# GATB/leon

Hardware: AMD Instinct MI355X
Metric: compressed input MB/s (DNA encode path) (higher is better)
Workload: dtype u64

## Files before the change

### leon_amd/csrc/capi.hip

```cpp
#include "../../include/leon_dna.h"
#include "kernels.h"
#include "host_rc.h"
#include "staging.h"
#include "host_blocks.h"

#include "prim.h"

#include <algorithm>
#include <atomic>
#include <chrono>
#include <cstdio>
#include <cstdlib>
#include <cstring>
#include <functional>
#include <mutex>
#include <string>
#include <thread>
#include <vector>

using namespace leon;

namespace {

thread_local std::string g_create_error;
// ... 820 lines not shown
            if (int rc = resolve_window(w0, w1)) return rc;
            while (w1 < n && packed_upto < std::min(n, w1 + W)) { if (int rc = pack_next_group()) return rc; }
            c->stats.resolve_windows++;
        }
        if (pending.buf >= 0) { HIPCHK(c, spin_sync(s)); hand_over(); }
        if (knobs.trace_resolve) {
            unsigned long long t[12];
            HIPCHK(c, hipMemcpy(t, d_trace, sizeof t, hipMemcpyDeviceToHost));
            const char* cls[3] = {"found an anchor of the dictionary", "went on to propose its own", "no anchor at all"};
            for (int j = 0; j < 3; j++)
                if (t[4 * j]) fprintf(stderr, "[leon resolve] k_lookup_cand, reads that %-34s: %10llu reads, per read %.1f filter probes, %.1f dictionary probes behind a filter maybe, %.1f k-mers through the bloom\n",
                                      cls[j], t[4 * j], (double)t[4 * j + 1] / t[4 * j], (double)t[4 * j + 2] / t[4 * j], (double)t[4 * j + 3] / t[4 * j]);
        }
        HIPCHK(c, hipGetLastError());
        HIPCHK(c, hipEventRecord(c->ev[2], s));
        mark("resolution launched to its end");
        return LEON_OK;
    }
    int resolve_window(uint64_t w0, uint64_t w1) {
        if (int rc = dict_reserve(c, c->n_keys + (w1 - w0))) return rc;
        HIPCHK(c, hipMemsetAsync(counters, 0, 8, s));
        HIPCHK(c, hipMemsetAsync(c->wbits.p, 0, (1ull << WBITS_LOG2) / 8, s));
        HIPCHK(c, hipMemsetAsync(c->pbits.p, 0, (1ull << WBITS_LOG2) / 8, s));
        if (!share_lookups) launch_lookup_cand(s, R, c->B, c->d_rv16, c->D, V, w0, w1, first_read_index, lists[0], counters, d_trace);
        else if (int rc = look_up_shared(w0, w1)) return rc;
        HIPCHK(c, hipMemcpyAsync(d_hist, counters, 4, hipMemcpyDeviceToDevice, s));
        uint32_t cnt0 = 0;
        if (int rc = fixpoint_rounds(w0, w1, cnt0)) return rc;
        hint = std::max<uint32_t>(2 * cnt0, 4096);
        if (cnt0 > 0) { if (int rc = settle(w0, w1)) return rc; }
        launch_finalize_reads(s, R, c->D, V, w0, w1);
        return LEON_OK;
    }
    int look_up_shared(uint64_t w0, uint64_t w1) {
        const uint32_t Wn = c->shard_world; const uint64_t P = (w1 - w0 + Wn - 1) / Wn;
        auto run_of = [&](uint32_t r, uint64_t& a, uint64_t& b) { a = std::min(w1, w0 + (uint64_t)r * P); b = std::min(w1, a + P); };
        HIPCHK(c, c->xch_res.ensure((uint64_t)Wn * P * 8)); uint64_t* xres = c->xch_res.as<uint64_t>();
        uint64_t s0 = 0, s1 = 0; run_of(c->shard_rank, s0, s1);
        launch_lookup_cand(s, R, c->B, c->d_rv16, c->D, V, s0, s1, first_read_index, lists[0], counters, d_trace, xres, w0, false);
        HIPCHK(c, hipStreamSynchronize(s));
        const auto t_l0 = std::chrono::steady_clock::now();
        if (c->xch_mode == LEON_XCH_BY_ANCHOR) {
            if (c->gather_fn(c->gather_user, xres, P * 8, Wn)) return fail(c, LEON_E_STATE, "the gather callback returned non-zero");
            HIPCHK(c, hipSetDevice(c->device));
            lk_call_ms += ms_since(t_l0);
        } else {
            for (uint32_t r = 0; r < Wn; r++) {
                if (r == c->shard_rank) continue;
                uint64_t a = 0, b = 0; run_of(r, a, b);
                launch_lookup_cand(s, R, c->B, c->d_rv16, c->D, V, a, b, first_read_index, lists[0], counters, nullptr, xres, w0, true);
            }
            HIPCHK(c, hipStreamSynchronize(s));
            lk_emul_ms += ms_since(t_l0);
        }
        launch_lookup_apply(s, R, c->D, V, w0, w1, s0, s1, first_read_index, xres, lists[0], counters);
        return LEON_OK;
    }
    int fixpoint_rounds(uint64_t w0, uint64_t w1, uint32_t& cnt0) {
        int cur = 0;
        uint32_t n_hist = 1;
        bool first_wait = true;
        for (uint32_t ahead = knobs.rounds_ahead;; ahead = kRoundsMore) {
            for (uint32_t r = 0; r < ahead && n_hist < kHist; r++) {
                const int nxt = cur ^ 1;
                const uint32_t h = std::max<uint32_t>(hint >> (2 * (n_hist - 1) < 31 ? 2 * (n_hist - 1) : 31), 4096);
                HIPCHK(c, hipMemsetAsync(counters + nxt, 0, 4, s));
                launch_check(s, R, c->D, V, first_read_index, lists[cur], counters + cur, h, lists[nxt], counters + nxt);
                HIPCHK(c, hipMemcpyAsync(d_hist + n_hist, counters + nxt, 4, hipMemcpyDeviceToDevice, s));
                launch_reset_tent(s, c->D, V, lists[cur], counters + cur, h);
                launch_propose(s, c->D, V, first_read_index, lists[nxt], counters + nxt, h);
                cur = nxt; n_hist++;
            }
            HIPCHK(c, hipMemcpyAsync(c->h_rb + 8, d_hist, n_hist * 4, hipMemcpyDeviceToHost, s));
// ... 51 lines not shown
            launch_chain_prep(s, true, R, c->D, V, first_read_index, w0, clist + c0, nc, c0, rank, cnt, own, rows, ent, om, late, dep, xdep);
            if (launch_chain_seq(s, nc, cnt, own, dep, xdep, rows, ent, c->chain_ins.as<unsigned long long>(), d_ctrace))
                return fail(c, LEON_E_HIP, "the sequential resolution pass could not be launched (its LDS request was refused)");
            launch_chain_apply(s, c->D, V, first_read_index, clist + c0, nc, c->chain_ins.as<unsigned long long>(), k);
            HIPCHK(c, hipGetLastError());
        }
        { const uint32_t c_last = (left - 1) / CH * CH; launch_chain_repropose(s, c->D, V, first_read_index, clist + c_last, left - c_last, nullptr, 0); }
        HIPCHK(c, hipEventRecord(c->chain_ev[2 * n_chain_ev + 1], s));
        n_chain_ev++;
        c->stats.resolve_chain_reads += left; c->stats.resolve_chain_windows++;
        if (knobs.trace_chain) {
            unsigned long long t[8];
            HIPCHK(c, hipStreamSynchronize(s));
            HIPCHK(c, hipMemcpy(t, d_ctrace, sizeof t, hipMemcpyDeviceToHost));
            float cms = 0; (void)hipEventElapsedTime(&cms, c->chain_ev[2 * n_chain_ev - 2], c->chain_ev[2 * n_chain_ev - 1]);
            fprintf(stderr, "[leon chain] window [%llu, %llu): %u reads left by the rounds; %llu steps of 64, %.2f ballot iterations and %.1f entry rows per step, %llu inserters; %.2f ms; per step the settler waited %.0f (tester: %.0f), settled + published %.0f ticks of s_memtime\n",
                    (unsigned long long)w0, (unsigned long long)w1, left, t[0], t[0] ? (double)t[1] / t[0] : 0.0, t[0] ? (double)t[2] / t[0] : 0.0, t[3], cms,
                    t[0] ? (double)t[4] / t[0] : 0.0, t[0] ? (double)t[5] / t[0] : 0.0, t[0] ? (double)t[6] / t[0] : 0.0);
        }
        return LEON_OK;
    }
    int settle(uint64_t w0, uint64_t w1) {
        launch_final_pos(s, R, c->D, V, w0, w1, first_read_index);
        launch_ins_flags(s, V, w0, w1);
        HIPCHK(c, prim::ExclusiveSum(c->cub_tmp.p, scan_tmp, V.ins_flag, c->rank.as<uint32_t>(), w1 - w0, s));
        HIPCHK(c, hipMemcpyAsync(c->h_rb + 0, c->rank.as<uint32_t>() + (w1 - w0 - 1), 4, hipMemcpyDeviceToHost, s));
        HIPCHK(c, hipMemcpyAsync(c->h_rb + 1, V.ins_flag + (w1 - w0 - 1), 4, hipMemcpyDeviceToHost, s));
        HIPCHK(c, hipMemcpyAsync(c->h_rb + 2, c->d_nkeys, 8, hipMemcpyDeviceToHost, s));
        HIPCHK(c, spin_sync(s));
        const uint64_t n_new = (uint64_t)(uint32_t)c->h_rb[0] + (uint32_t)c->h_rb[1];
        c->n_keys = c->h_rb[2];
        if (c->n_anchors + n_new > 0xFFFFFFFFull) return fail(c, LEON_E_OVERFLOW, "more than 2^32 anchors");
        if ((c->n_anchors + n_new) * 8 * KW > c->anchor_kmers.cap) {
            TmpBuf nb;
            HIPCHK(c, nb.ensure(std::max<uint64_t>((c->n_anchors + n_new) * 2, 1024) * 8 * KW));
            if (c->n_anchors) HIPCHK(c, hipMemcpyAsync(nb.p, c->anchor_kmers.p, c->n_anchors * 8 * KW, hipMemcpyDeviceToDevice, s));
            HIPCHK(c, hipStreamSynchronize(s));
            std::swap(static_cast<DevBuf&>(nb).p, c->anchor_kmers.p);
            std::swap(static_cast<DevBuf&>(nb).cap, c->anchor_kmers.cap);
        }
        launch_assign_addr(s, c->D, V, w0, w1, c->rank.as<uint32_t>(), c->n_anchors, c->anchor_kmers.as<uint64_t>(), k);
        if (n_new && c->shard_rank == 0 && !(c->cfg.flags & LEON_F_DICT_ON_DEVICE)) {
            HIPCHK(c, hipMemcpyAsync(c->h_anchor[anchor_buf], c->anchor_kmers.as<uint64_t>() + c->n_anchors * KW, n_new * 8 * KW, hipMemcpyDeviceToHost, s));
            pending.buf = anchor_buf; pending.n = n_new;
            anchor_buf ^= 1;
            if (w0 == 0) {
                HIPCHK(c, spin_sync(s));
// ... 1263 lines not shown
```

### leon_amd/csrc/dna_kernels.hip

```cpp
#include "kernels.h"

namespace leon {

static inline uint32_t grid_for(uint64_t items, uint32_t per_block, uint32_t cap = 256 * 32) {
    uint64_t g = (items + per_block - 1) / per_block;
    if (g < 1) g = 1;
    if (g > cap) g = cap;
    return (uint32_t)g;
}
#define DISPATCH_K(k, CALL) do { if ((k) >= 32) { typedef u128 K; CALL; } else { typedef uint64_t K; CALL; } } while (0)

template <typename K>
__global__ void __launch_bounds__(256) k_bloom_insert(BloomDev B, const uint16_t* rv16g, const uint64_t* kmers, uint64_t n) {
    __shared__ uint16_t rv16[256];
    load_rv16(rv16, rv16g);
    uint32_t* words = (uint32_t*)B.bits;
    for (uint64_t i = blockIdx.x * (uint64_t)blockDim.x + threadIdx.x; i < n; i += (uint64_t)gridDim.x * blockDim.x) {
        BloomKeys Kk;
        const uint32_t pv = bloom_item_keys<K>(B, rv16, load_kmer<K>(kmers + i * KT<K>::W), Kk);
        for (uint32_t h = 0; h < B.n_hash; h++) {
            uint64_t pos = Kk.racine + Kk.key[h] + pv;
            atomicOr(&words[pos >> 5], 1u << (pos & 31));
        }
    }
// ... 256 lines not shown
template <typename K> __device__ inline K canon_at(const uint32_t* pk, uint32_t p, uint32_t k) {
    const K km = kmer_at<K>(pk, p, k);
    const K rc = revcomp(km, k);
    return rc < km ? rc : km;
}

template <typename K> __device__ inline K fwd_from_words16(uint32_t words, uint32_t gbase, uint32_t base, uint32_t p, uint32_t k);
template <> __device__ inline uint64_t fwd_from_words16<uint64_t>(uint32_t words, uint32_t gbase, uint32_t base, uint32_t p, uint32_t k) {
    const int d = (int)(gbase + (p >> 4) - (base >> 4));
    return kmer_from3((uint32_t)__shfl((int)words, d), (uint32_t)__shfl((int)words, d + 1), (uint32_t)__shfl((int)words, d + 2), p & 15, k);
}
template <> __device__ inline u128 fwd_from_words16<u128>(uint32_t words, uint32_t gbase, uint32_t base, uint32_t p, uint32_t k) {
    const int d = (int)(gbase + (p >> 4) - (base >> 4));
    return kmer_from5((uint32_t)__shfl((int)words, d), (uint32_t)__shfl((int)words, d + 1), (uint32_t)__shfl((int)words, d + 2),
                      (uint32_t)__shfl((int)words, d + 3), (uint32_t)__shfl((int)words, d + 4), p & 15, k);
}
template <typename K> __device__ inline K canon_from_words16(uint32_t words, uint32_t gbase, uint32_t base, uint32_t p, uint32_t k) {
    const K km = fwd_from_words16<K>(words, gbase, base, p, k);
    const K rc = revcomp(km, k);
    return rc < km ? rc : km;
}

template <typename K, bool TRACE>
__global__ void __launch_bounds__(256, (KT<K>::W == 2 ? 5 : 8)) k_lookup_cand(ReadsDev R, BloomDev B, const uint16_t* rv16g, DictDev D, ResolveDev V,
                                                    uint64_t w0, uint64_t w1, uint64_t first_global,
                                                    uint32_t* ulist, uint32_t* ucount, unsigned long long* trace,
                                                    uint64_t* xres, uint64_t xbase, uint32_t dry) {
    __shared__ uint16_t rv16[256];
    load_rv16(rv16, rv16g);
    const uint32_t lane = lane_id(), k = R.k;
    const uint32_t grp = lane >> 4, l = lane & 15, gbase = grp * 16;
    const uint64_t wave = (blockIdx.x * (uint64_t)blockDim.x + threadIdx.x) >> 6;
    const uint64_t nwaves = ((uint64_t)gridDim.x * blockDim.x) >> 6;
    enum : uint32_t { PH_LOOKUP = 0, PH_SEG_A = 1, PH_SEG_B = 2, PH_SEG_C = 3, PH_DONE = 4 };
    __shared__ uint32_t lists[4][64];
    uint32_t* my_list = lists[threadIdx.x >> 6];
    uint32_t n_list = 0, n_created = 0;
    auto flush_list = [&]() {
        if (n_list) {
            uint32_t at = 0;
            if (lane == 0) at = atomicAdd(ucount, n_list);
            at = (uint32_t)__shfl((int)at, 0);
            __builtin_amdgcn_wave_barrier();
            if (lane < n_list) ulist[at + lane] = my_list[lane];
            __builtin_amdgcn_wave_barrier();
        }
        if (n_created && lane == 0) atomicAdd(D.n_keys, (unsigned long long)n_created);
        n_list = 0; n_created = 0;
    };
    uint32_t t_filter = 0, t_dict = 0, t_bloom = 0;
    unsigned long long tr[12] = {0, 0, 0, 0, 0, 0, 0, 0, 0, 0, 0, 0};
    auto trace_done = [&](uint32_t cls) { if (TRACE && l == 0) { tr[cls * 4] += 1; tr[cls * 4 + 1] += t_filter; tr[cls * 4 + 2] += t_dict; tr[cls * 4 + 3] += t_bloom; } t_filter = t_dict = t_bloom = 0; };
    uint64_t i = w0 + 4 * wave + grp;
    bool have = false, started = false, exhausted = false;
    uint32_t len = 0, nk = 0, iMin = 0, iMax = 0, phase = PH_DONE, base = 0, limit = 0;
    uint64_t g = 0;
    const uint32_t* pk = R.packed;
    const uint32_t mm_m = D.mm_m, mm_P = D.mm_P, mm_c = D.mm_c;
    const uint64_t* const fwords = (const uint64_t*)D.fbits;
    MinLevels prev = {~0u, ~0u, ~0u, ~0u, ~0u};
    for (;;) {
        if (phase == PH_DONE && !exhausted) {
            if (started) i += 4 * nwaves;
            started = true;
            have = i < w1;
            exhausted = !have;
            if (have) {
                len = R.len[i];
                g = first_global + i;
                pk = R.packed + 2 * R.slot_off[i];
                nk = len >= k ? len - k + 1 : 0;
                iMin = nk / 2; iMax = nk / 2 + 10 > nk ? nk : nk / 2 + 10;
                base = 0; limit = nk;
                if (nk) phase = PH_LOOKUP;
                else { if (l == 0) { if (!dry) V.status[i] = ST_NOANCHOR; if (xres) xres[i - xbase] = ST_NOANCHOR; } trace_done(2); }
            }
        }
        if (!__any(have)) break;
        {
            const bool active = phase != PH_DONE;
            if (active && base >= limit) {
                if (phase == PH_LOOKUP) { phase = PH_SEG_A; base = iMin; limit = iMax; }
                else if (phase == PH_SEG_A) { phase = PH_SEG_B; base = 0; limit = iMin; }
                else if (phase == PH_SEG_B) { phase = PH_SEG_C; base = iMax; limit = nk; }
                else { phase = PH_DONE; if (l == 0) { if (!dry) V.status[i] = ST_NOANCHOR; if (xres) xres[i - xbase] = ST_NOANCHOR; } trace_done(2); }
            }
            const bool run = phase != PH_DONE && base < limit;
            const uint32_t p = base + l;
            const bool valid = run && p < limit;
            const uint32_t words = (run && l < 8) ? pk[(base >> 4) + l] : 0u;
            const K km = fwd_from_words16<K>(words, gbase, base, valid ? p : (run ? limit - 1 : 0), k);
            const K rck = revcomp(km, k);
            const K cn = rck < km ? rck : km;
            const bool look = run && phase == PH_LOOKUP;
            if (look && base == 0) {
                prev = MinLevels{~0u, ~0u, ~0u, ~0u, ~0u};
                for (int r = mm_P == 32 ? 1 : 0; r >= 0; r--) {
                    const int x = (int)(mm_c + mm_P - 1) - 16 * (r + 1) + (int)l;
                    const uint32_t xc = x > 0 ? (uint32_t)x : 0u;
                    const uint32_t w0 = (uint32_t)__shfl((int)words, (int)(gbase + (xc >> 4))), w1 = (uint32_t)__shfl((int)words, (int)(gbase + (xc >> 4) + 1));
                    const uint32_t mm = (uint32_t)((((((uint64_t)w0) << 32) | w1) << (2 * (xc & 15))) >> (64 - 2 * mm_m));
                    prev = sliding_levels(x >= (int)mm_c && xc + mm_m <= len ? mmer_hash(mm, mm_m) : ~0u, prev);
                }
            }
            const MinLevels cur = sliding_levels(look && valid ? mmer_hash(mmer_of(km, k, mm_m, mm_c + mm_P - 1), mm_m) : ~0u, prev);
            const uint32_t hmin = window_minimum(cur, prev, mm_P);
            if (look) prev = cur;
            bool hit = false; uint32_t slot = 0xFFFFFFFFu;
            if (valid) {
                if (phase == PH_LOOKUP) {
                    const uint64_t fb = filter_bits(cn);
                    const bool maybe = (fwords[filter_word(D, hmin)] & fb) == fb;
                    if (maybe) { uint64_t fin = IDX_INF; slot = dict_find(D, cn, fin); hit = slot != 0xFFFFFFFFu && fin < g; }
                    if (TRACE) {
                        const uint32_t nf = (uint32_t)__popcll(__ballot(true) >> gbase & 0xFFFFull), nd = (uint32_t)__popcll(__ballot(maybe) >> gbase & 0xFFFFull);
                        t_filter += nf; t_dict += nd;
                    }
                }
                else { hit = bloom_contains<K>(B, rv16, cn); if (TRACE) t_bloom += (uint32_t)__popcll(__ballot(true) >> gbase & 0xFFFFull); }
            }
            const unsigned long long bal = __ballot(hit);
            const uint32_t gb = (uint32_t)(bal >> gbase) & 0xFFFFu;
            bool want_insert = false; uint32_t cpos = 0;
            if (run) {
                if (gb) {
                    const uint32_t f = (uint32_t)__builtin_ctz(gb);
                    const uint32_t hs = __shfl(slot, (int)(gbase + f));
                    if (phase == PH_LOOKUP) {
                        if (l == 0) {
                            if (!dry) { V.status[i] = ST_HIT; V.hit_pos[i] = base + f; V.hit_slot[i] = hs; }
                            if (xres) xres[i - xbase] = ((uint64_t)(base + f) << 8) | ST_HIT;
                        }
                        trace_done(0);
                    } else {
                        want_insert = (l == 0) && !dry; cpos = base + f;
                        if (l == 0 && xres) xres[i - xbase] = ((uint64_t)cpos << 8) | ST_UNRESOLVED;
                        trace_done(1);
                    }
                    phase = PH_DONE;
                } else base += 16;
            }
            bool created = false;
            uint32_t sl = 0;
            for (uint32_t q = 0; q < 4; q++) {
                if (want_insert && grp == q) {
                    const K ck = canon_at<K>(pk, cpos, k);
                    sl = dict_find_or_insert<true>(D, ck, created);
                    atomicMin((unsigned long long*)tent_ptr(D, sl), (unsigned long long)g);
                    const uint32_t pb = window_bit(ck);
                    atomicOr(&D.pbits[pb >> 5], 1u << (pb & 31));
                    V.status[i] = ST_UNRESOLVED; V.cand_pos[i] = cpos; V.cand_slot[i] = sl;
                }
            }
            const unsigned long long wm = __ballot(want_insert);
            if (wm) {
                if (want_insert) my_list[n_list + (uint32_t)__popcll(wm & ((1ull << lane) - 1))] = (uint32_t)i;
                n_list += (uint32_t)__popcll(wm);
                n_created += (uint32_t)__popcll(__ballot(created));
                if (n_list > 64 - 4) flush_list();
            }
        }
    }
    flush_list();
    if (TRACE) {
        for (uint32_t j = 0; j < 12; j++) {
            unsigned long long v = tr[j];
            for (int d = 1; d < 64; d <<= 1) v += __shfl_xor(v, d);
            if (lane == 0 && v) atomicAdd(trace + j, v);
        }
    }
}
void launch_lookup_cand(hipStream_t s, ReadsDev R, BloomDev B, const uint16_t* rv16, DictDev D, ResolveDev V,
                        uint64_t w0, uint64_t w1, uint64_t first_global, uint32_t* ulist, uint32_t* ucount, unsigned long long* trace,
                        uint64_t* xres, uint64_t xbase, bool dry) {
    if (w1 <= w0) return;
    if (trace && !dry) { DISPATCH_K(R.k, hipLaunchKernelGGL((k_lookup_cand<K, true>), dim3(grid_for(w1 - w0, 16, 256 * 16)), dim3(256), 0, s, R, B, rv16, D, V, w0, w1,
                                                           first_global, ulist, ucount, trace, xres, xbase, 0u)); return; }
    const uint32_t per_cu = [] { const char* e = getenv("LEON_LOOKUP_BLOCKS_PER_CU"); const int v = e ? atoi(e) : 0; return v > 0 && v <= 1024 ? (uint32_t)v : 16u; }();
    DISPATCH_K(R.k, hipLaunchKernelGGL((k_lookup_cand<K, false>), dim3(grid_for(w1 - w0, 16, 256 * per_cu)), dim3(256), 0, s, R, B, rv16, D, V, w0, w1,
                                       first_global, ulist, ucount, trace, xres, xbase, dry ? 1u : 0u));
}

template <typename K>
__global__ void __launch_bounds__(256) k_lookup_apply(ReadsDev R, DictDev D, ResolveDev V, uint64_t w0, uint64_t w1, uint64_t s0, uint64_t s1,
                                                     uint64_t first_global, const uint64_t* xres, uint32_t* ulist, uint32_t* ucount) {
    __shared__ uint32_t wave_n[4], wave_new[4], block_at;
    const uint32_t lane = lane_id(), wv = threadIdx.x >> 6, k = R.k;
    const uint64_t before = s0 - w0, n_out = (w1 - w0) - (s1 - s0);
    for (uint64_t e0 = blockIdx.x * (uint64_t)blockDim.x; e0 < n_out; e0 += (uint64_t)gridDim.x * blockDim.x) {
        const uint64_t e = e0 + threadIdx.x;
        const bool have = e < n_out;
        const uint64_t i = !have ? w0 : (e < before ? w0 + e : s1 + (e - before));
        const uint64_t x = have ? xres[i - w0] : (uint64_t)ST_NOANCHOR;
        const uint32_t st = (uint32_t)(x & 0xFFu), pos = (uint32_t)(x >> 8);
        const uint64_t g = first_global + i;
        const uint32_t* pk = R.packed + 2 * R.slot_off[i];
        const bool sane = have && (st == ST_NOANCHOR || ((st == ST_HIT || st == ST_UNRESOLVED) && R.len[i] >= k && pos <= R.len[i] - k));
        if (have && !sane) atomicExch(D.err, 2);
        if (sane && st == ST_NOANCHOR) V.status[i] = ST_NOANCHOR;
        if (sane && st == ST_HIT) {
            uint64_t fin = IDX_INF;
            const uint32_t slot = dict_find(D, canon_at<K>(pk, pos, k), fin);
            if (slot == 0xFFFFFFFFu || !(fin < g)) atomicExch(D.err, 2);
// ... 144 lines not shown
    uint32_t n = *count;
    for (uint64_t e = blockIdx.x * (uint64_t)blockDim.x + threadIdx.x; e < n; e += (uint64_t)gridDim.x * blockDim.x) {
        uint32_t i = list[e];
        atomicMin((unsigned long long*)tent_ptr(D, V.cand_slot[i]), (unsigned long long)(first_global + i));
    }
}
void launch_propose(hipStream_t s, DictDev D, ResolveDev V, uint64_t first_global, const uint32_t* list,
                    const uint32_t* count, uint32_t max_count) {
    if (!max_count) return;
    hipLaunchKernelGGL(k_propose, dim3(grid_for(max_count, 256)), dim3(256), 0, s, D, V, first_global, list, count);
}

template <typename K>
__global__ void __launch_bounds__(256) k_final_pos(ReadsDev R, DictDev D, ResolveDev V, uint64_t w0, uint64_t w1, uint64_t first_global) {
    const uint32_t lane = lane_id(), k = R.k;
    const uint32_t grp = lane >> 4, l = lane & 15, gbase = grp * 16;
    const uint64_t wave = (blockIdx.x * (uint64_t)blockDim.x + threadIdx.x) >> 6;
    const uint64_t nwaves = ((uint64_t)gridDim.x * blockDim.x) >> 6;
    for (uint64_t i0 = w0 + 4 * wave; i0 < w1; i0 += 4 * nwaves) {
        const uint64_t i = i0 + grp;
        const bool have = i < w1;
        const uint8_t st = have ? V.status[i] : (uint8_t)ST_NOANCHOR;
        const bool mine = st == ST_HIT || st == ST_HITNEW;
        const uint64_t g = first_global + i;
        const uint32_t limit = !mine ? 0u : (st == ST_HIT ? V.hit_pos[i] : R.len[i] - k + 1);
        const uint32_t* pk = R.packed + 2 * (mine ? R.slot_off[i] : 0);
        uint32_t base = 0;
        bool done = limit == 0;
        while (__any(!done)) {
            const bool run = !done;
            const uint32_t p = base + l;
            const bool valid = run && p < limit;
            const uint32_t words = (run && l < 8) ? pk[(base >> 4) + l] : 0u;
            const K cn = canon_from_words16<K>(words, gbase, base, valid ? p : (run ? limit - 1 : 0), k);
            bool hit = false; uint32_t slot = 0xFFFFFFFFu;
            if (valid) {
                const uint32_t wb = window_bit(cn);
                if ((D.wbits[wb >> 5] >> (wb & 31)) & 1u) {
                    uint64_t fin = IDX_INF;
                    slot = dict_find(D, cn, fin);
                    hit = slot != 0xFFFFFFFFu && fin < g;
                }
            }
            const unsigned long long bal = __ballot(hit);
            const uint32_t gb = (uint32_t)(bal >> gbase) & 0xFFFFu;
            if (run) {
                if (gb) {
                    const uint32_t f = (uint32_t)__builtin_ctz(gb);
                    const uint32_t hs = __shfl(slot, (int)(gbase + f));
                    if (l == 0) { V.hit_pos[i] = base + f; V.hit_slot[i] = hs; }
                    done = true;
                } else { base += 16; done = base >= limit; }
            }
        }
    }
}
void launch_final_pos(hipStream_t s, ReadsDev R, DictDev D, ResolveDev V, uint64_t w0, uint64_t w1, uint64_t first_global) {
    if (w1 <= w0) return;
    DISPATCH_K(R.k, hipLaunchKernelGGL(k_final_pos<K>, dim3(grid_for(w1 - w0, 16, 256 * 16)), dim3(256), 0, s, R, D, V, w0, w1, first_global));
}

__global__ void k_ins_flags(ResolveDev V, uint64_t w0, uint64_t w1) {
    for (uint64_t i = w0 + blockIdx.x * (uint64_t)blockDim.x + threadIdx.x; i < w1; i += (uint64_t)gridDim.x * blockDim.x)
        V.ins_flag[i - w0] = V.status[i] == ST_INSERTER ? 1u : 0u;
}
void launch_ins_flags(hipStream_t s, ResolveDev V, uint64_t w0, uint64_t w1) {
    if (w1 <= w0) return;
    hipLaunchKernelGGL(k_ins_flags, dim3(grid_for(w1 - w0, 256)), dim3(256), 0, s, V, w0, w1);
}
template <typename K>
__global__ void k_assign_addr(DictDev D, ResolveDev V, uint64_t w0, uint64_t w1, const uint32_t* rank, uint64_t addr_base,
                              uint64_t* anchor_kmers) {
    for (uint64_t i = w0 + blockIdx.x * (uint64_t)blockDim.x + threadIdx.x; i < w1; i += (uint64_t)gridDim.x * blockDim.x) {
        if (V.status[i] != ST_INSERTER) continue;
        uint64_t a = addr_base + rank[i - w0];
        uint32_t slot = V.cand_slot[i];
        D.addr[slot] = (uint32_t)a;
        store_kmer(anchor_kmers + a * KT<K>::W, dict_key<K>(D, slot));
        V.hit_pos[i] = V.cand_pos[i];
        V.hit_slot[i] = slot;
    }
}
void launch_assign_addr(hipStream_t s, DictDev D, ResolveDev V, uint64_t w0, uint64_t w1, const uint32_t* rank,
                        uint64_t addr_base, uint64_t* anchor_kmers, uint32_t k) {
    if (w1 <= w0) return;
    DISPATCH_K(k, hipLaunchKernelGGL(k_assign_addr<K>, dim3(grid_for(w1 - w0, 256)), dim3(256), 0, s, D, V, w0, w1, rank, addr_base, anchor_kmers));
}
template <typename K>
__global__ void k_finalize_reads(ReadsDev R, DictDev D, ResolveDev V, uint64_t w0, uint64_t w1) {
    uint32_t k = R.k;
    for (uint64_t i = w0 + blockIdx.x * (uint64_t)blockDim.x + threadIdx.x; i < w1; i += (uint64_t)gridDim.x * blockDim.x) {
        uint8_t st = V.status[i];
// ... 988 lines not shown
```

### leon_amd/csrc/kernels.h

```cpp
#pragma once
#include <hip/hip_runtime.h>
#include <stdint.h>
#include "leon_device.h"

namespace leon {

struct ReadsDev {
    const uint32_t* packed;
    const uint32_t* nmask;
    const uint64_t* slot_off;
    const uint64_t* base_off;
    const uint32_t* len;
    const uint32_t* n_count;
    uint64_t n;
    uint64_t ev_origin;
    uint32_t k, pad;
};

struct DictDev {
    uint64_t* slots;
    uint64_t* tent;
    uint64_t tstride;
    uint32_t* addr;
    uint64_t mask;
// ... 18 lines not shown
constexpr uint32_t FBITS_LOG2_MAX = 31;
constexpr uint32_t FBITS_LOG2_DEFAULT = 28;

enum : uint8_t { ST_NOANCHOR = 0, ST_HIT = 1, ST_UNRESOLVED = 2, ST_INSERTER = 3, ST_HITNEW = 4 };

struct ResolveDev {
    uint8_t* status;
    uint32_t* hit_pos; uint32_t* hit_slot;
    uint32_t* cand_pos; uint32_t* cand_slot;
    int32_t* anchor_pos; uint32_t* anchor_addr; uint8_t* flags; uint64_t* sort_key;
    uint32_t* ins_flag;
};

void launch_bloom_insert(hipStream_t s, BloomDev B, const uint16_t* rv16, const uint64_t* kmers, uint64_t n);
void launch_bloom_query(hipStream_t s, BloomDev B, const uint16_t* rv16, const uint64_t* kmers, uint64_t n,
                        int mode , uint8_t* out);
void launch_rebase_offsets(hipStream_t s, uint64_t* off, uint64_t n, uint64_t base);
void launch_read_slots(hipStream_t s, const uint64_t* base_off, uint64_t n, uint64_t* slots, uint32_t* bad );
void launch_pack(hipStream_t s, const uint8_t* bases, const uint64_t* base_off, const uint64_t* slot_off, uint64_t n,
                 uint32_t* packed, uint32_t* nmask, uint32_t* len, uint32_t* n_count);
void launch_dict_init(hipStream_t s, DictDev D, uint64_t cap, uint32_t W);
void launch_dict_rehash(hipStream_t s, DictDev from, uint64_t from_cap, DictDev to, uint32_t k);
void launch_lookup_cand(hipStream_t s, ReadsDev R, BloomDev B, const uint16_t* rv16, DictDev D, ResolveDev V,
                        uint64_t w0, uint64_t w1, uint64_t first_global, uint32_t* ulist, uint32_t* ucount,
                        unsigned long long* trace = nullptr ,
                        uint64_t* xres = nullptr ,
                        uint64_t xbase = 0, bool dry = false );
void launch_lookup_apply(hipStream_t s, ReadsDev R, DictDev D, ResolveDev V, uint64_t w0, uint64_t w1, uint64_t s0, uint64_t s1,
                         uint64_t first_global, const uint64_t* xres, uint32_t* ulist, uint32_t* ucount);
void launch_check(hipStream_t s, ReadsDev R, DictDev D, ResolveDev V, uint64_t first_global,
                  const uint32_t* ulist, const uint32_t* ucount, uint32_t max_count, uint32_t* next_list, uint32_t* next_count);
void launch_reset_tent(hipStream_t s, DictDev D, ResolveDev V, const uint32_t* list, const uint32_t* count, uint32_t max_count);
void launch_propose(hipStream_t s, DictDev D, ResolveDev V, uint64_t first_global, const uint32_t* list,
                    const uint32_t* count, uint32_t max_count);
void launch_final_pos(hipStream_t s, ReadsDev R, DictDev D, ResolveDev V, uint64_t w0, uint64_t w1, uint64_t first_global);
void launch_ins_flags(hipStream_t s, ResolveDev V, uint64_t w0, uint64_t w1);
void launch_assign_addr(hipStream_t s, DictDev D, ResolveDev V, uint64_t w0, uint64_t w1, const uint32_t* rank,
                        uint64_t addr_base, uint64_t* anchor_kmers, uint32_t k);
constexpr uint32_t CHAIN_LOG2 = 19;
constexpr uint32_t CHAIN_EL = 96;
constexpr uint32_t CHAIN_DEPTH = 3;
void launch_chain_flags(hipStream_t s, ResolveDev V, uint64_t w0, uint64_t w1, uint32_t* flag);
void launch_chain_compact(hipStream_t s, ResolveDev V, uint64_t w0, uint64_t w1, const uint32_t* rank, uint32_t* list);
void launch_chain_repropose(hipStream_t s, DictDev D, ResolveDev V, uint64_t first_global, const uint32_t* reset_list, uint32_t n_reset,
                            const uint32_t* list, uint32_t n);
void launch_chain_prep(hipStream_t s, bool fill, ReadsDev R, DictDev D, ResolveDev V, uint64_t first_global, uint64_t w0, const uint32_t* list,
                       uint32_t n, uint32_t c0, const uint32_t* rank, uint32_t* cnt, uint32_t* own, const uint64_t* gbase, uint32_t* ent,
                       const unsigned long long* om, const unsigned long long* late, unsigned long long* dep, unsigned long long* xdep);
void launch_chain_tables(hipStream_t s, const uint32_t* cnt, const uint32_t* own, uint32_t n, uint64_t* rows ,
                         unsigned long long* om , unsigned long long* late );
int launch_chain_seq(hipStream_t s, uint32_t n, const uint32_t* cnt, const uint32_t* own, const unsigned long long* dep, const unsigned long long* xdep,
                     const uint64_t* gbase, const uint32_t* ent, unsigned long long* ins , unsigned long long* trace );
void launch_chain_apply(hipStream_t s, DictDev D, ResolveDev V, uint64_t first_global, const uint32_t* list, uint32_t n, const unsigned long long* ins, uint32_t k);
void launch_anchor_symbols(hipStream_t s, const uint64_t* kmers, uint64_t n_anchors, uint32_t k, uint8_t* syms);
void launch_finalize_reads(hipStream_t s, ReadsDev R, DictDev D, ResolveDev V, uint64_t w0, uint64_t w1);
struct WalkCache { uint64_t* slots; uint64_t bucket_mask; uint32_t hop_shift, pad; };
void launch_walk_cache_init(hipStream_t s, WalkCache C, uint32_t k);
void launch_walk(hipStream_t s, ReadsDev R, BloomDev B, const uint16_t* rv16, const int32_t* anchor_pos, const uint8_t* flags,
                 const uint32_t* perm, uint64_t n_walk, uint8_t* events, const uint64_t* ev_off = nullptr ,
// ... 86 lines not shown
```

Baseline: 18800.

## Split anchor lookup and bloom proposal into two kernels with a compacted pending list

The single lookup kernel that ran dictionary lookup and then bloom-based candidate proposal per read is split in two. The first kernel only does the filter and dictionary lookup and appends reads without a hit to a compacted pending list. The second kernel walks only those pending reads with a configurable lanes-per-read width, so divergent reads no longer hold up lookup waves. Separately, the ins_flag computation is folded into k_final_pos, which removes one kernel launch. The cost is an extra launch, a memset, and a pending list sized by the previous window's hint; if the hint undercounts, that list could be too small.

```diff
diff --git a/leon_amd/csrc/capi.hip b/leon_amd/csrc/capi.hip
--- a/leon_amd/csrc/capi.hip
+++ b/leon_amd/csrc/capi.hip
@@ -866,7 +866,7 @@
         HIPCHK(c, hipMemsetAsync(counters, 0, 8, s));
         HIPCHK(c, hipMemsetAsync(c->wbits.p, 0, (1ull << WBITS_LOG2) / 8, s));
         HIPCHK(c, hipMemsetAsync(c->pbits.p, 0, (1ull << WBITS_LOG2) / 8, s));
-        if (!share_lookups) launch_lookup_cand(s, R, c->B, c->d_rv16, c->D, V, w0, w1, first_read_index, lists[0], counters, d_trace);
+        if (!share_lookups) launch_lookup_cand(s, R, c->B, c->d_rv16, c->D, V, w0, w1, first_read_index, lists[1], counters + 2, hint, lists[0], counters, d_trace);
         else if (int rc = look_up_shared(w0, w1)) return rc;
         HIPCHK(c, hipMemcpyAsync(d_hist, counters, 4, hipMemcpyDeviceToDevice, s));
         uint32_t cnt0 = 0;
@@ -881,7 +881,7 @@
         auto run_of = [&](uint32_t r, uint64_t& a, uint64_t& b) { a = std::min(w1, w0 + (uint64_t)r * P); b = std::min(w1, a + P); };
         HIPCHK(c, c->xch_res.ensure((uint64_t)Wn * P * 8)); uint64_t* xres = c->xch_res.as<uint64_t>();
         uint64_t s0 = 0, s1 = 0; run_of(c->shard_rank, s0, s1);
-        launch_lookup_cand(s, R, c->B, c->d_rv16, c->D, V, s0, s1, first_read_index, lists[0], counters, d_trace, xres, w0, false);
+        launch_lookup_cand(s, R, c->B, c->d_rv16, c->D, V, s0, s1, first_read_index, lists[1], counters + 2, hint, lists[0], counters, d_trace, xres, w0, false);
         HIPCHK(c, hipStreamSynchronize(s));
         const auto t_l0 = std::chrono::steady_clock::now();
         if (c->xch_mode == LEON_XCH_BY_ANCHOR) {
@@ -892,7 +892,7 @@
             for (uint32_t r = 0; r < Wn; r++) {
                 if (r == c->shard_rank) continue;
                 uint64_t a = 0, b = 0; run_of(r, a, b);
-                launch_lookup_cand(s, R, c->B, c->d_rv16, c->D, V, a, b, first_read_index, lists[0], counters, nullptr, xres, w0, true);
+                launch_lookup_cand(s, R, c->B, c->d_rv16, c->D, V, a, b, first_read_index, lists[1], counters + 2, hint, lists[0], counters, nullptr, xres, w0, true);
             }
             HIPCHK(c, hipStreamSynchronize(s));
             lk_emul_ms += ms_since(t_l0);
@@ -990,7 +990,6 @@
     }
     int settle(uint64_t w0, uint64_t w1) {
         launch_final_pos(s, R, c->D, V, w0, w1, first_read_index);
-        launch_ins_flags(s, V, w0, w1);
         HIPCHK(c, prim::ExclusiveSum(c->cub_tmp.p, scan_tmp, V.ins_flag, c->rank.as<uint32_t>(), w1 - w0, s));
         HIPCHK(c, hipMemcpyAsync(c->h_rb + 0, c->rank.as<uint32_t>() + (w1 - w0 - 1), 4, hipMemcpyDeviceToHost, s));
         HIPCHK(c, hipMemcpyAsync(c->h_rb + 1, V.ins_flag + (w1 - w0 - 1), 4, hipMemcpyDeviceToHost, s));
diff --git a/leon_amd/csrc/dna_kernels.hip b/leon_amd/csrc/dna_kernels.hip
--- a/leon_amd/csrc/dna_kernels.hip
+++ b/leon_amd/csrc/dna_kernels.hip
@@ -302,17 +302,137 @@
 }
 
 template <typename K, bool TRACE>
-__global__ void __launch_bounds__(256, (KT<K>::W == 2 ? 5 : 8)) k_lookup_cand(ReadsDev R, BloomDev B, const uint16_t* rv16g, DictDev D, ResolveDev V,
+__global__ void __launch_bounds__(256, (KT<K>::W == 2 ? 5 : 8)) k_lookup_cand(ReadsDev R, DictDev D, ResolveDev V,
                                                     uint64_t w0, uint64_t w1, uint64_t first_global,
-                                                    uint32_t* ulist, uint32_t* ucount, unsigned long long* trace,
+                                                    uint32_t* plist, uint32_t* pcount, unsigned long long* trace,
                                                     uint64_t* xres, uint64_t xbase, uint32_t dry) {
-    __shared__ uint16_t rv16[256];
-    load_rv16(rv16, rv16g);
     const uint32_t lane = lane_id(), k = R.k;
     const uint32_t grp = lane >> 4, l = lane & 15, gbase = grp * 16;
     const uint64_t wave = (blockIdx.x * (uint64_t)blockDim.x + threadIdx.x) >> 6;
     const uint64_t nwaves = ((uint64_t)gridDim.x * blockDim.x) >> 6;
-    enum : uint32_t { PH_LOOKUP = 0, PH_SEG_A = 1, PH_SEG_B = 2, PH_SEG_C = 3, PH_DONE = 4 };
+    __shared__ uint32_t lists[4][64];
+    uint32_t* my_list = lists[threadIdx.x >> 6];
+    uint32_t n_list = 0;
+    auto flush_list = [&]() {
+        if (!n_list) return;
+        uint32_t at = 0;
+        if (lane == 0) at = atomicAdd(pcount, n_list);
+        at = (uint32_t)__shfl((int)at, 0);
+        __builtin_amdgcn_wave_barrier();
+        if (lane < n_list) plist[at + lane] = my_list[lane];
+        __builtin_amdgcn_wave_barrier();
+        n_list = 0;
+    };
+    uint32_t t_filter = 0, t_dict = 0;
+    unsigned long long tr[12] = {0, 0, 0, 0, 0, 0, 0, 0, 0, 0, 0, 0};
+    auto trace_done = [&](uint32_t cls) { if (TRACE && l == 0) { tr[cls * 4] += 1; tr[cls * 4 + 1] += t_filter; tr[cls * 4 + 2] += t_dict; } t_filter = t_dict = 0; };
+    uint64_t i = w0 + 4 * wave + grp;
+    bool have = false, started = false, exhausted = false, busy = false;
+    uint32_t len = 0, nk = 0, base = 0;
+    uint64_t g = 0;
+    const uint32_t* pk = R.packed;
+    const uint32_t mm_m = D.mm_m, mm_P = D.mm_P, mm_c = D.mm_c;
+    const uint64_t* const fwords = (const uint64_t*)D.fbits;
+    MinLevels prev = {~0u, ~0u, ~0u, ~0u, ~0u};
+    for (;;) {
+        if (!busy && !exhausted) {
+            if (started) i += 4 * nwaves;
+            started = true;
+            have = i < w1;
+            exhausted = !have;
+            if (have) {
+                len = R.len[i];
+                g = first_global + i;
+                pk = R.packed + 2 * R.slot_off[i];
+                nk = len >= k ? len - k + 1 : 0;
+                base = 0;
+                if (nk) busy = true;
+                else { if (l == 0) { if (!dry) V.status[i] = ST_NOANCHOR; if (xres) xres[i - xbase] = ST_NOANCHOR; } trace_done(2); }
+            }
+        }
+        if (!__any(have)) break;
+        {
+            const bool run = busy;
+            const uint32_t p = base + l;
+            const bool valid = run && p < nk;
+            const uint32_t words = (run && l < 8) ? pk[(base >> 4) + l] : 0u;
+            const K km = fwd_from_words16<K>(words, gbase, base, valid ? p : (run ? nk - 1 : 0), k);
+            const K rck = revcomp(km, k);
+            const K cn = rck < km ? rck : km;
+            if (run && base == 0) {
+                prev = MinLevels{~0u, ~0u, ~0u, ~0u, ~0u};
+                for (int r = mm_P == 32 ? 1 : 0; r >= 0; r--) {
+                    const int x = (int)(mm_c + mm_P - 1) - 16 * (r + 1) + (int)l;
+                    const uint32_t xc = x > 0 ? (uint32_t)x : 0u;
+                    const uint32_t w0 = (uint32_t)__shfl((int)words, (int)(gbase + (xc >> 4))), w1 = (uint32_t)__shfl((int)words, (int)(gbase + (xc >> 4) + 1));
+                    const uint32_t mm = (uint32_t)((((((uint64_t)w0) << 32) | w1) << (2 * (xc & 15))) >> (64 - 2 * mm_m));
+                    prev = sliding_levels(x >= (int)mm_c && xc + mm_m <= len ? mmer_hash(mm, mm_m) : ~0u, prev);
+                }
+            }
+            const MinLevels cur = sliding_levels(valid ? mmer_hash(mmer_of(km, k, mm_m, mm_c + mm_P - 1), mm_m) : ~0u, prev);
+            const uint32_t hmin = window_minimum(cur, prev, mm_P);
+            if (run) prev = cur;
+            bool hit = false; uint32_t slot = 0xFFFFFFFFu;
+            if (valid) {
+                const uint64_t fb = filter_bits(cn);
+                const bool maybe = (fwords[filter_word(D, hmin)] & fb) == fb;
+                if (maybe) { uint64_t fin = IDX_INF; slot = dict_find(D, cn, fin); hit = slot != 0xFFFFFFFFu && fin < g; }
+                if (TRACE) {
+                    const uint32_t nf = (uint32_t)__popcll(__ballot(true) >> gbase & 0xFFFFull), nd = (uint32_t)__popcll(__ballot(maybe) >> gbase & 0xFFFFull);
+                    t_filter += nf; t_dict += nd;
+                }
+            }
+            const unsigned long long bal = __ballot(hit);
+            const uint32_t gb = (uint32_t)(bal >> gbase) & 0xFFFFu;
+            bool pend = false;
+            if (run) {
+                if (gb) {
+                    const uint32_t f = (uint32_t)__builtin_ctz(gb);
+                    const uint32_t hs = __shfl(slot, (int)(gbase + f));
+                    if (l == 0) {
+                        if (!dry) { V.status[i] = ST_HIT; V.hit_pos[i] = base + f; V.hit_slot[i] = hs; }
+                        if (xres) xres[i - xbase] = ((uint64_t)(base + f) << 8) | ST_HIT;
+                    }
+                    trace_done(0);
+                    busy = false;
+                } else {
+                    base += 16;
+                    if (base >= nk) {
+                        busy = false; pend = l == 0;
+                        if (TRACE) { if (l == 0) { V.cand_pos[i] = t_filter; V.cand_slot[i] = t_dict; } t_filter = t_dict = 0; }
+                    }
+                }
+            }
+            const unsigned long long wm = __ballot(pend);
+            if (wm) {
+                if (pend) my_list[n_list + (uint32_t)__popcll(wm & ((1ull << lane) - 1))] = (uint32_t)i;
+                n_list += (uint32_t)__popcll(wm);
+                if (n_list > 64 - 4) flush_list();
+            }
+        }
+    }
+    flush_list();
+    if (TRACE) {
+        for (uint32_t j = 0; j < 12; j++) {
+            unsigned long long v = tr[j];
+            for (int d = 1; d < 64; d <<= 1) v += __shfl_xor(v, d);
+            if (lane == 0 && v) atomicAdd(trace + j, v);
+        }
+    }
+}
+
+template <typename K, uint32_t LPR, bool TRACE>
+__global__ void __launch_bounds__(256) k_propose_cand(ReadsDev R, BloomDev B, const uint16_t* rv16g, DictDev D, ResolveDev V, uint64_t first_global,
+                                                     const uint32_t* plist, const uint32_t* pcount, uint32_t* ulist, uint32_t* ucount,
+                                                     unsigned long long* trace, uint64_t* xres, uint64_t xbase, uint32_t dry) {
+    __shared__ uint16_t rv16[256];
+    load_rv16(rv16, rv16g);
+    constexpr uint32_t RPW = 64 / LPR, GMASK = (uint32_t)((1ull << LPR) - 1);
+    const uint32_t lane = lane_id(), k = R.k;
+    const uint32_t grp = lane / LPR, l = lane % LPR, gbase = grp * LPR;
+    const uint64_t wave = (blockIdx.x * (uint64_t)blockDim.x + threadIdx.x) >> 6;
+    const uint64_t nwaves = ((uint64_t)gridDim.x * blockDim.x) >> 6;
+    const uint32_t count = *pcount;
     __shared__ uint32_t lists[4][64];
     uint32_t* my_list = lists[threadIdx.x >> 6];
     uint32_t n_list = 0, n_created = 0;
@@ -331,114 +451,71 @@
     uint32_t t_filter = 0, t_dict = 0, t_bloom = 0;
     unsigned long long tr[12] = {0, 0, 0, 0, 0, 0, 0, 0, 0, 0, 0, 0};
     auto trace_done = [&](uint32_t cls) { if (TRACE && l == 0) { tr[cls * 4] += 1; tr[cls * 4 + 1] += t_filter; tr[cls * 4 + 2] += t_dict; tr[cls * 4 + 3] += t_bloom; } t_filter = t_dict = t_bloom = 0; };
-    uint64_t i = w0 + 4 * wave + grp;
-    bool have = false, started = false, exhausted = false;
-    uint32_t len = 0, nk = 0, iMin = 0, iMax = 0, phase = PH_DONE, base = 0, limit = 0;
-    uint64_t g = 0;
+    uint64_t e = RPW * wave + grp;
+    bool have = false, started = false, exhausted = false, busy = false;
+    uint32_t i = 0, nk = 0, iMin = 0, iMax = 0, seg = 0, base = 0, limit = 0;
     const uint32_t* pk = R.packed;
-    const uint32_t mm_m = D.mm_m, mm_P = D.mm_P, mm_c = D.mm_c;
-    const uint64_t* const fwords = (const uint64_t*)D.fbits;
-    MinLevels prev = {~0u, ~0u, ~0u, ~0u, ~0u};
     for (;;) {
-        if (phase == PH_DONE && !exhausted) {
-            if (started) i += 4 * nwaves;
+        if (!busy && !exhausted) {
+            if (started) e += RPW * nwaves;
             started = true;
-            have = i < w1;
+            have = e < count;
             exhausted = !have;
             if (have) {
-                len = R.len[i];
-                g = first_global + i;
+                i = plist[e];
                 pk = R.packed + 2 * R.slot_off[i];
-                nk = len >= k ? len - k + 1 : 0;
+                nk = R.len[i] - k + 1;
                 iMin = nk / 2; iMax = nk / 2 + 10 > nk ? nk : nk / 2 + 10;
-                base = 0; limit = nk;
-                if (nk) phase = PH_LOOKUP;
-                else { if (l == 0) { if (!dry) V.status[i] = ST_NOANCHOR; if (xres) xres[i - xbase] = ST_NOANCHOR; } trace_done(2); }
+                seg = 0; base = iMin; limit = iMax;
+                busy = true;
+                if (TRACE && l == 0) { t_filter = V.cand_pos[i]; t_dict = V.cand_slot[i]; }
             }
         }
         if (!__any(have)) break;
-        {
-            const bool active = phase != PH_DONE;
-            if (active && base >= limit) {
-                if (phase == PH_LOOKUP) { phase = PH_SEG_A; base = iMin; limit = iMax; }
-                else if (phase == PH_SEG_A) { phase = PH_SEG_B; base = 0; limit = iMin; }
-                else if (phase == PH_SEG_B) { phase = PH_SEG_C; base = iMax; limit = nk; }
-                else { phase = PH_DONE; if (l == 0) { if (!dry) V.status[i] = ST_NOANCHOR; if (xres) xres[i - xbase] = ST_NOANCHOR; } trace_done(2); }
-            }
-            const bool run = phase != PH_DONE && base < limit;
-            const uint32_t p = base + l;
-            const bool valid = run && p < limit;
-            const uint32_t words = (run && l < 8) ? pk[(base >> 4) + l] : 0u;
-            const K km = fwd_from_words16<K>(words, gbase, base, valid ? p : (run ? limit - 1 : 0), k);
-            const K rck = revcomp(km, k);
-            const K cn = rck < km ? rck : km;
-            const bool look = run && phase == PH_LOOKUP;
-            if (look && base == 0) {
-                prev = MinLevels{~0u, ~0u, ~0u, ~0u, ~0u};
-                for (int r = mm_P == 32 ? 1 : 0; r >= 0; r--) {
-                    const int x = (int)(mm_c + mm_P - 1) - 16 * (r + 1) + (int)l;
-                    const uint32_t xc = x > 0 ? (uint32_t)x : 0u;
-                    const uint32_t w0 = (uint32_t)__shfl((int)words, (int)(gbase + (xc >> 4))), w1 = (uint32_t)__shfl((int)words, (int)(gbase + (xc >> 4) + 1));
-                    const uint32_t mm = (uint32_t)((((((uint64_t)w0) << 32) | w1) << (2 * (xc & 15))) >> (64 - 2 * mm_m));
-                    prev = sliding_levels(x >= (int)mm_c && xc + mm_m <= len ? mmer_hash(mm, mm_m) : ~0u, prev);
-                }
-            }
-            const MinLevels cur = sliding_levels(look && valid ? mmer_hash(mmer_of(km, k, mm_m, mm_c + mm_P - 1), mm_m) : ~0u, prev);
-            const uint32_t hmin = window_minimum(cur, prev, mm_P);
-            if (look) prev = cur;
-            bool hit = false; uint32_t slot = 0xFFFFFFFFu;
-            if (valid) {
-                if (phase == PH_LOOKUP) {
-                    const uint64_t fb = filter_bits(cn);
-                    const bool maybe = (fwords[filter_word(D, hmin)] & fb) == fb;
-                    if (maybe) { uint64_t fin = IDX_INF; slot = dict_find(D, cn, fin); hit = slot != 0xFFFFFFFFu && fin < g; }
-                    if (TRACE) {
-                        const uint32_t nf = (uint32_t)__popcll(__ballot(true) >> gbase & 0xFFFFull), nd = (uint32_t)__popcll(__ballot(maybe) >> gbase & 0xFFFFull);
-                        t_filter += nf; t_dict += nd;
-                    }
-                }
-                else { hit = bloom_contains<K>(B, rv16, cn); if (TRACE) t_bloom += (uint32_t)__popcll(__ballot(true) >> gbase & 0xFFFFull); }
-            }
-            const unsigned long long bal = __ballot(hit);
-            const uint32_t gb = (uint32_t)(bal >> gbase) & 0xFFFFu;
-            bool want_insert = false; uint32_t cpos = 0;
-            if (run) {
-                if (gb) {
-                    const uint32_t f = (uint32_t)__builtin_ctz(gb);
-                    const uint32_t hs = __shfl(slot, (int)(gbase + f));
-                    if (phase == PH_LOOKUP) {
-                        if (l == 0) {
-                            if (!dry) { V.status[i] = ST_HIT; V.hit_pos[i] = base + f; V.hit_slot[i] = hs; }
-                            if (xres) xres[i - xbase] = ((uint64_t)(base + f) << 8) | ST_HIT;
-                        }
-                        trace_done(0);
-                    } else {
-                        want_insert = (l == 0) && !dry; cpos = base + f;
-                        if (l == 0 && xres) xres[i - xbase] = ((uint64_t)cpos << 8) | ST_UNRESOLVED;
-                        trace_done(1);
-                    }
-                    phase = PH_DONE;
-                } else base += 16;
-            }
-            bool created = false;
-            uint32_t sl = 0;
-            for (uint32_t q = 0; q < 4; q++) {
-                if (want_insert && grp == q) {
-                    const K ck = canon_at<K>(pk, cpos, k);
-                    sl = dict_find_or_insert<true>(D, ck, created);
-                    atomicMin((unsigned long long*)tent_ptr(D, sl), (unsigned long long)g);
-                    const uint32_t pb = window_bit(ck);
-                    atomicOr(&D.pbits[pb >> 5], 1u << (pb & 31));
-                    V.status[i] = ST_UNRESOLVED; V.cand_pos[i] = cpos; V.cand_slot[i] = sl;
-                }
-            }
-            const unsigned long long wm = __ballot(want_insert);
-            if (wm) {
-                if (want_insert) my_list[n_list + (uint32_t)__popcll(wm & ((1ull << lane) - 1))] = (uint32_t)i;
-                n_list += (uint32_t)__popcll(wm);
-                n_created += (uint32_t)__popcll(__ballot(created));
-                if (n_list > 64 - 4) flush_list();
-            }
+        if (busy && seg == 0 && base >= limit) { seg = 1; base = 0; limit = iMin; }
+        if (busy && seg == 1 && base >= limit) { seg = 2; base = iMax; limit = nk; }
+        if (busy && seg == 2 && base >= limit) {
+            busy = false;
+            if (l == 0) { if (!dry) V.status[i] = ST_NOANCHOR; if (xres) xres[i - xbase] = ST_NOANCHOR; }
+            trace_done(2);
+        }
+        const bool run = busy;
+        const uint32_t p = base + l;
+        const bool valid = run && p < limit;
+        bool hit = false;
+        if (valid) hit = bloom_contains<K>(B, rv16, canon_at<K>(pk, p, k));
+        if (TRACE) t_bloom += (uint32_t)__popcll((__ballot(valid) >> gbase) & GMASK);
+        const uint32_t gb = (uint32_t)(__ballot(hit) >> gbase) & GMASK;
+        bool want_insert = false; uint32_t cpos = 0;
+        if (run) {
+            if (gb) {
+                cpos = base + (uint32_t)__builtin_ctz(gb);
+                want_insert = (l == 0) && !dry;
+                if (l == 0 && xres) xres[i - xbase] = ((uint64_t)cpos << 8) | ST_UNRESOLVED;
+                trace_done(1);
+                busy = false;
+            } else base += LPR;
+        }
+        bool created = false;
+        auto propose = [&]() {
+            const uint64_t g = first_global + i;
+            const K ck = canon_at<K>(pk, cpos, k);
+            const uint32_t sl = dict_find_or_insert<true>(D, ck, created);
+            atomicMin((unsigned long long*)tent_ptr(D, sl), (unsigned long long)g);
+            const uint32_t pb = window_bit(ck);
+            atomicOr(&D.pbits[pb >> 5], 1u << (pb & 31));
+            V.status[i] = ST_UNRESOLVED; V.cand_pos[i] = cpos; V.cand_slot[i] = sl;
+        };
+        const unsigned long long wm = __ballot(want_insert);
+        if (wm) {
+            if (KT<K>::W == 1) { if (want_insert) propose(); }
+            else {
+                for (unsigned long long m = wm; m; m &= m - 1) if (lane == (uint32_t)__builtin_ctzll(m)) propose();
+            }
+            if (want_insert) my_list[n_list + (uint32_t)__popcll(wm & ((1ull << lane) - 1))] = i;
+            n_list += (uint32_t)__popcll(wm);
+            n_created += (uint32_t)__popcll(__ballot(created));
+            if (n_list > 64 - RPW) flush_list();
         }
     }
     flush_list();
@@ -450,15 +527,32 @@
         }
     }
 }
+template <typename K>
+static void lookup_then_propose(hipStream_t s, ReadsDev R, BloomDev B, const uint16_t* rv16, DictDev D, ResolveDev V, uint64_t w0, uint64_t w1,
+                                uint64_t first_global, uint32_t* plist, uint32_t* pcount, uint32_t max_pending, uint32_t* ulist, uint32_t* ucount,
+                                unsigned long long* trace, uint64_t* xres, uint64_t xbase, bool dry) {
+    const uint32_t dr = dry ? 1u : 0u;
+    const bool traced = trace && !dry;
+    const uint32_t per_cu = [] { const char* e = getenv("LEON_LOOKUP_BLOCKS_PER_CU"); const int v = e ? atoi(e) : 0; return v > 0 && v <= 1024 ? (uint32_t)v : 16u; }();
+    const uint32_t lanes = [] { const char* e = getenv("LEON_PROPOSE_LANES"); const int v = e ? atoi(e) : 0; return v == 8 || v == 16 ? (uint32_t)v : 4u; }();
+    const dim3 grid_a(grid_for(w1 - w0, 16, 256 * (traced ? 16 : per_cu)));
+    const dim3 grid_b(grid_for(max_pending, 4 * (64 / lanes), 256 * (traced ? 16 : per_cu)));
+    if (traced) {
+        hipLaunchKernelGGL((k_lookup_cand<K, true>), grid_a, dim3(256), 0, s, R, D, V, w0, w1, first_global, plist, pcount, trace, xres, xbase, 0u);
+        hipLaunchKernelGGL((k_propose_cand<K, 4, true>), dim3(grid_for(max_pending, 64, 256 * 16)), dim3(256), 0, s, R, B, rv16, D, V, first_global, plist, pcount, ulist, ucount, trace, xres, xbase, 0u);
+        return;
+    }
+    hipLaunchKernelGGL((k_lookup_cand<K, false>), grid_a, dim3(256), 0, s, R, D, V, w0, w1, first_global, plist, pcount, trace, xres, xbase, dr);
+#define LEON_PROPOSE(LPR) hipLaunchKernelGGL((k_propose_cand<K, LPR, false>), grid_b, dim3(256), 0, s, R, B, rv16, D, V, first_global, plist, pcount, ulist, ucount, trace, xres, xbase, dr)
+    if (lanes == 16) LEON_PROPOSE(16); else if (lanes == 8) LEON_PROPOSE(8); else LEON_PROPOSE(4);
+#undef LEON_PROPOSE
+}
 void launch_lookup_cand(hipStream_t s, ReadsDev R, BloomDev B, const uint16_t* rv16, DictDev D, ResolveDev V,
-                        uint64_t w0, uint64_t w1, uint64_t first_global, uint32_t* ulist, uint32_t* ucount, unsigned long long* trace,
-                        uint64_t* xres, uint64_t xbase, bool dry) {
+                        uint64_t w0, uint64_t w1, uint64_t first_global, uint32_t* plist, uint32_t* pcount, uint32_t max_pending,
+                        uint32_t* ulist, uint32_t* ucount, unsigned long long* trace, uint64_t* xres, uint64_t xbase, bool dry) {
     if (w1 <= w0) return;
-    if (trace && !dry) { DISPATCH_K(R.k, hipLaunchKernelGGL((k_lookup_cand<K, true>), dim3(grid_for(w1 - w0, 16, 256 * 16)), dim3(256), 0, s, R, B, rv16, D, V, w0, w1,
-                                                           first_global, ulist, ucount, trace, xres, xbase, 0u)); return; }
-    const uint32_t per_cu = [] { const char* e = getenv("LEON_LOOKUP_BLOCKS_PER_CU"); const int v = e ? atoi(e) : 0; return v > 0 && v <= 1024 ? (uint32_t)v : 16u; }();
-    DISPATCH_K(R.k, hipLaunchKernelGGL((k_lookup_cand<K, false>), dim3(grid_for(w1 - w0, 16, 256 * per_cu)), dim3(256), 0, s, R, B, rv16, D, V, w0, w1,
-                                       first_global, ulist, ucount, trace, xres, xbase, dry ? 1u : 0u));
+    (void)hipMemsetAsync(pcount, 0, 4, s);
+    DISPATCH_K(R.k, lookup_then_propose<K>(s, R, B, rv16, D, V, w0, w1, first_global, plist, pcount, max_pending, ulist, ucount, trace, xres, xbase, dry));
 }
 
 template <typename K>
@@ -649,6 +743,7 @@
         const bool have = i < w1;
         const uint8_t st = have ? V.status[i] : (uint8_t)ST_NOANCHOR;
         const bool mine = st == ST_HIT || st == ST_HITNEW;
+        if (have && l == 0) V.ins_flag[i - w0] = st == ST_INSERTER ? 1u : 0u;
         const uint64_t g = first_global + i;
         const uint32_t limit = !mine ? 0u : (st == ST_HIT ? V.hit_pos[i] : R.len[i] - k + 1);
         const uint32_t* pk = R.packed + 2 * (mine ? R.slot_off[i] : 0);
@@ -687,14 +782,6 @@
     DISPATCH_K(R.k, hipLaunchKernelGGL(k_final_pos<K>, dim3(grid_for(w1 - w0, 16, 256 * 16)), dim3(256), 0, s, R, D, V, w0, w1, first_global));
 }
 
-__global__ void k_ins_flags(ResolveDev V, uint64_t w0, uint64_t w1) {
-    for (uint64_t i = w0 + blockIdx.x * (uint64_t)blockDim.x + threadIdx.x; i < w1; i += (uint64_t)gridDim.x * blockDim.x)
-        V.ins_flag[i - w0] = V.status[i] == ST_INSERTER ? 1u : 0u;
-}
-void launch_ins_flags(hipStream_t s, ResolveDev V, uint64_t w0, uint64_t w1) {
-    if (w1 <= w0) return;
-    hipLaunchKernelGGL(k_ins_flags, dim3(grid_for(w1 - w0, 256)), dim3(256), 0, s, V, w0, w1);
-}
 template <typename K>
 __global__ void k_assign_addr(DictDev D, ResolveDev V, uint64_t w0, uint64_t w1, const uint32_t* rank, uint64_t addr_base,
                               uint64_t* anchor_kmers) {
diff --git a/leon_amd/csrc/kernels.h b/leon_amd/csrc/kernels.h
--- a/leon_amd/csrc/kernels.h
+++ b/leon_amd/csrc/kernels.h
@@ -64,7 +64,8 @@
 void launch_dict_init(hipStream_t s, DictDev D, uint64_t cap, uint32_t W);
 void launch_dict_rehash(hipStream_t s, DictDev from, uint64_t from_cap, DictDev to, uint32_t k);
 void launch_lookup_cand(hipStream_t s, ReadsDev R, BloomDev B, const uint16_t* rv16, DictDev D, ResolveDev V,
-                        uint64_t w0, uint64_t w1, uint64_t first_global, uint32_t* ulist, uint32_t* ucount,
+                        uint64_t w0, uint64_t w1, uint64_t first_global, uint32_t* plist, uint32_t* pcount, uint32_t max_pending,
+                        uint32_t* ulist, uint32_t* ucount,
                         unsigned long long* trace = nullptr ,
                         uint64_t* xres = nullptr ,
                         uint64_t xbase = 0, bool dry = false );
@@ -76,7 +77,6 @@
 void launch_propose(hipStream_t s, DictDev D, ResolveDev V, uint64_t first_global, const uint32_t* list,
                     const uint32_t* count, uint32_t max_count);
 void launch_final_pos(hipStream_t s, ReadsDev R, DictDev D, ResolveDev V, uint64_t w0, uint64_t w1, uint64_t first_global);
-void launch_ins_flags(hipStream_t s, ResolveDev V, uint64_t w0, uint64_t w1);
 void launch_assign_addr(hipStream_t s, DictDev D, ResolveDev V, uint64_t w0, uint64_t w1, const uint32_t* rank,
                         uint64_t addr_base, uint64_t* anchor_kmers, uint32_t k);
 constexpr uint32_t CHAIN_LOG2 = 19;
```

Result: no change. 18660 (-0.8%).
